# XuanchenLi/Topo4D

Measured on AMD Instinct MI355X. Metric: rasterizer fwd+bwd views/sec, higher is better.
Workload: dtype f32

## Files before the change

topo4d_amd/csrc/t4d_raster.hip:

```cpp
#include <hip/hip_runtime.h>
#include <stdint.h>
#include <stdio.h>
#include <stdlib.h>
#include <string.h>
#include <vector>

#include "../../include/t4d_config.h"
#include "../../include/topo4d_raster.h"
#include "t4d_activations.h"

#define T4D_EXPORT extern "C" __attribute__((visibility("default")))

namespace {

constexpr int kBlock = 256;
#ifndef T4D_FWD_BATCH
#define T4D_FWD_BATCH 192
#endif
constexpr int kFwdBatch = T4D_FWD_BATCH;
#ifndef T4D_BWD_BATCH
#define T4D_BWD_BATCH 128
#endif
constexpr int kBwdBatch = T4D_BWD_BATCH;
constexpr int kSortLdsCap = 2048;
constexpr int kLongBlock = 1024;
constexpr int kScanChunk = 1024;
constexpr int kRankSortMax = 512;
constexpr int kHist = 1024;
constexpr int kBuckets = 24;
constexpr int kGP = T4D_GRAD_PAIR_FLOATS;
constexpr int kCursorSegs = 64;
#ifndef T4D_SEG
// ... 108 lines not shown
    unsigned long long *keys, *sort_tmp;
    float *cut_r2;
    float *final_T;
    uint32_t *n_contrib;
    float *out_color, *out_depth, *out_alpha;
    int32_t *radii;
    const float *dL_dcolor, *dL_ddepth, *dL_dalpha;
    float *grad_pair;
    float *dL_dmeans3D, *dL_dmeans2D, *dL_dcolors, *dL_dshs, *dL_dopacities, *dL_dscales, *dL_drotations, *dL_dcov3D;
    float *tile_dot;
    float *cotangent_dot;
    uint32_t tile_blocks;
    uint32_t fill_blocks;
    uint32_t fill_vec;
    uint4 *slot_tab;
    float *snap;
    uint32_t slots_per_view;
    uint32_t fused_sort;
    unsigned long long *host_status;
    uint32_t seg_min_pairs;
    uint32_t *live;
    uint32_t slots_by_offset;
    uint32_t views_per_set;
};

__device__ __forceinline__ float ndc2pix(float v, int S)
{
#pragma clang fp contract(off)
    return ((v + 1.0f) * S - 1.0f) * 0.5f;
}

__device__ __forceinline__ void tile_rect(float px, float py, int r, int gx, int gy, int &x0, int &y0, int &x1, int &y1)
{
    x0 = min(gx, max(0, (int)((px - r) / T4D_TILE_X)));
    y0 = min(gy, max(0, (int)((py - r) / T4D_TILE_Y)));
    x1 = min(gx, max(0, (int)((px + r + T4D_TILE_X - 1) / T4D_TILE_X)));
    y1 = min(gy, max(0, (int)((py + r + T4D_TILE_Y - 1) / T4D_TILE_Y)));
}

typedef const __attribute__((address_space(4))) float *const_float_p;
struct ViewRecord {
    float view[16], proj[16], campos[3], bg[3], tanx, tany;
};
__device__ __forceinline__ ViewRecord load_view_record(const float *views, const int v)
{
    const_float_p p = (const_float_p)(views + (size_t)v * T4D_VIEW_FLOATS);
    ViewRecord r;
// ... 294 lines not shown
    kp.cut_r2 = reinterpret_cast<float *>(st + L.pair_rank);
    kp.tile_off = reinterpret_cast<uint32_t *>(st + L.tile_off);
    kp.chunk_sum = reinterpret_cast<uint32_t *>(st + L.chunk_sum);
    kp.n_chunks = (kp.T + kScanChunk - 1) / kScanChunk;
    kp.long_bins_elsewhere = (p.flags & T4D_FLAG_NO_LONG_BINS) ? 0 : 1;
    kp.pair_off = reinterpret_cast<uint32_t *>(st + L.pair_off);
    kp.xy = reinterpret_cast<float2 *>(st + L.xy);
    kp.depth = reinterpret_cast<float *>(st + L.depth);
    kp.conic_opacity = reinterpret_cast<float4 *>(st + L.conic_opacity);
    kp.rgb = reinterpret_cast<float *>(st + L.rgb);
    kp.clamped = reinterpret_cast<uint8_t *>(st + L.clamped);
    kp.keys = reinterpret_cast<unsigned long long *>(st + L.keys);
    kp.sort_tmp = reinterpret_cast<unsigned long long *>(st + L.sort_tmp);
    kp.final_T = reinterpret_cast<float *>(st + L.final_T);
    kp.n_contrib = reinterpret_cast<uint32_t *>(st + L.n_contrib);
    kp.slot_tab = reinterpret_cast<uint4 *>(st + L.slot_tab);
    kp.snap = reinterpret_cast<float *>(st + L.snap);
    kp.live = reinterpret_cast<uint32_t *>(st + L.live);
    kp.slots_per_view = seg_capable(p) ? (uint32_t)seg_slots_per_view(p, (size_t)kp.T) : 0u;
    kp.seg_shift = seg_positions(p) == 64 ? 6u : 7u;
    kp.slots_by_offset = seg_mode(p) == 2 ? 1u : 0u;
    kp.seg_min_pairs = seg_mode(p) == 2 ? ((p.flags & T4D_FLAG_NO_LONG_BINS) ? 0xffffffffu : (uint32_t)kSegLongMin) : 0u;
    static_assert(kSegOne == 64 && kSeg == 128, "seg_shift assumes segment lengths of 64 and 128");
}

}

T4D_EXPORT uint32_t t4d_abi_version(void) { return T4D_ABI_VERSION; }
T4D_EXPORT const char *t4d_last_error(void) { return g_err; }

T4D_EXPORT size_t t4d_state_bytes(const T4DProblem *prob)
{
    if (check_problem(prob) != T4D_OK) return 0;
    return make_layout(*prob).total;
}

size_t grad_pair_bytes(const T4DProblem &p) { return align_up((size_t)p.n_views * (size_t)p.pair_capacity * kGP * sizeof(float)); }
size_t tile_dot_bytes(const T4DProblem &p, size_t n_tiles) { return align_up((size_t)p.n_views * n_tiles * 4 * sizeof(float)); }

T4D_EXPORT size_t t4d_backward_scratch_bytes(const T4DProblem *prob)
{
    if (check_problem(prob) != T4D_OK) return 0;
    const size_t n_tiles = (size_t)((prob->W + T4D_TILE_X - 1) / T4D_TILE_X) * ((prob->H + T4D_TILE_Y - 1) / T4D_TILE_Y);
    return grad_pair_bytes(*prob) + tile_dot_bytes(*prob, n_tiles) +
           (prob->sh_coeffs > 0 ? align_up((size_t)prob->n_views * (size_t)prob->P * 3 * sizeof(float)) : 0);
}
// ... 36 lines not shown
{
    int rc = check_problem(prob);
    if (rc != T4D_OK) return rc;
    if (!io || !io->views || !io->means3D || !io->opacities || !io->out_color || !io->out_depth || !io->out_alpha ||
        !io->out_radii || !io->state)
        return fail(T4D_ERR_ARG, "null required pointer in T4DForwardIO");
    if ((io->shs == nullptr) == (io->colors_precomp == nullptr))
        return fail(T4D_ERR_ARG, "provide exactly one of shs / colors_precomp");
    if (io->cov3D_precomp ? (io->scales || io->rotations) : (!io->scales || !io->rotations))
        return fail(T4D_ERR_ARG, "provide exactly one of (scales, rotations) / cov3D_precomp");
    if (io->shs && prob->sh_coeffs < 1) return fail(T4D_ERR_ARG, "shs given but sh_coeffs == 0");
    T4DProblem p = *prob;
    if (!io->shs) p.sh_coeffs = 0;
    const Layout L = make_layout(p);
    if (io->state_bytes < L.total) return fail(T4D_ERR_STATE_SIZE, "state buffer smaller than t4d_state_bytes()");
    hipStream_t stream = (hipStream_t)hip_stream;
    const bool debug = (p.flags & T4D_FLAG_DEBUG_SYNC) != 0;
    const bool checked = debug || (p.flags & T4D_FLAG_CHECKED) != 0;
    char *st = (char *)io->state;

    KP kp;
    memset(&kp, 0, sizeof(kp));
    fill_common(kp, p, L, st);
    kp.views = io->views; kp.means3D = io->means3D; kp.opacities = io->opacities; kp.scales = io->scales;
    kp.rotations = io->rotations; kp.cov3D_precomp = io->cov3D_precomp; kp.colors_precomp = io->colors_precomp;
    kp.shs = io->shs;
    kp.out_color = io->out_color; kp.out_depth = io->out_depth; kp.out_alpha = io->out_alpha; kp.radii = io->out_radii;

    bool status_published = false;
    if (!checked && (p.flags & T4D_FLAG_ASYNC_STATUS) && status && p.n_views == 1 && kp.T <= kSmallTiles &&
        getenv("T4D_NO_SMALL_VIEW") == nullptr && getenv("T4D_STATUS_BY_COPY") == nullptr) {
        void *dptr = nullptr;
        if (hipHostGetDevicePointer(&dptr, (void *)status, 0) == hipSuccess && dptr != nullptr) {
            kp.host_status = (unsigned long long *)dptr;
            status_published = true;
        } else {
            (void)hipGetLastError();
        }
    }
    T4D_HIP(hipMemsetAsync(st, 0, L.zero_end, stream));
    const bool small_view = p.n_views == 1 && kp.T <= kSmallTiles && getenv("T4D_NO_SMALL_VIEW") == nullptr;
    const bool front = small_view && gaussian_grid(p.P, 1) + 1u <= 128u && gaussian_grid(p.P, 1) + 1u <= front_small_resident_blocks() &&
                       getenv("T4D_NO_FRONT_FUSION") == nullptr;
    { ProfScope ps_(stream, K_PREPROCESS);
    if (front) hipLaunchKernelGGL(k_front_small, dim3(gaussian_grid(p.P, 1) + 1), dim3(kBlock), 0, stream, kp);
    else hipLaunchKernelGGL(k_preprocess, dim3(gaussian_grid(p.P, p.n_views)), dim3(kBlock), 0, stream, kp);
// ... 32 lines not shown
    kp.fused_sort = (lat && (p.flags & T4D_FLAG_SHORT_BINS) != 0 && getenv("T4D_NO_FUSED_SORT") == nullptr) ? 1u : 0u;
    const bool long_fwd = kp.slots_per_view != 0u && kp.seg_min_pairs != 0xffffffffu && seg_mode(p) == 2 && !lat && getenv("T4D_NO_LONG_FWD") == nullptr;
    if (long_fwd && getenv("T4D_NO_FUSED_SORT") == nullptr) kp.fused_sort = 1u;
    if (!kp.fused_sort) {
        ProfScope ps_(stream, K_SORT_TILES);
        if (seg_mode(p) == 1 && (p.flags & T4D_FLAG_SHORT_BINS) == 0 && getenv("T4D_SORT_256") == nullptr)
            hipLaunchKernelGGL(k_sort_tiles<kLongBlock>, dim3(min(kp.T * p.n_views, 4 * device_cus())), dim3(kLongBlock), 0, stream, kp);
        else
            hipLaunchKernelGGL(k_sort_tiles<kBlock>, dim3(tile_grid(kp.T * p.n_views, 5, 2)), dim3(kBlock), 0, stream, kp);
    }
    T4D_LAUNCH_CHECK("k_sort_tiles");
    if (kp.long_bins_elsewhere) {
        ProfScope ps_(stream, K_SORT_LONG);
        hipLaunchKernelGGL(k_sort_long_chunks, dim3(min(kp.T * p.n_views, 2 * device_cus())), dim3(kLongBlock), 0, stream, kp);
        hipLaunchKernelGGL(k_merge_long, dim3(min(kp.T * p.n_views, 2 * device_cus())), dim3(kLongBlock), 0, stream, kp);
    }
    T4D_LAUNCH_CHECK("k_sort_long");
    {
    kp.tile_blocks = (uint32_t)(lat ? kp.T * p.n_views : tile_grid(kp.T * p.n_views, 6, 2));
    kp.fill_blocks = (uint32_t)(kp.gy * p.n_views);
    kp.fill_vec = (p.W % 4 == 0 && (((uintptr_t)io->out_color | (uintptr_t)io->out_depth | (uintptr_t)io->out_alpha) & 15u) == 0) ? 1u : 0u;
    if (getenv("T4D_FILL_SCALAR")) kp.fill_vec = 0u;
    const dim3 fgrid(kp.tile_blocks + kp.fill_blocks);
    const bool seg = kp.slots_per_view != 0u && kp.seg_min_pairs != 0xffffffffu;
    const bool seg_one = seg && seg_positions(p) == kSegOne;
    if (long_fwd) {
        { ProfScope ps_(stream, K_RENDER_FWD);
        hipLaunchKernelGGL((k_render_fwd<false, kFwdBatch, 0, true, true>), fgrid, dim3(kBlock), 0, stream, kp);
        }
        T4D_LAUNCH_CHECK("k_render_fwd");
        ProfScope psl_(stream, K_FWD_LONG);
        KP kl = kp;
        kl.tile_blocks = min(kp.slots_per_view, (uint32_t)(8 * device_cus()));
        hipLaunchKernelGGL(k_fwd_long_seg<false>, dim3(kl.tile_blocks), dim3(kBlock), 0, stream, kl);
        T4D_LAUNCH_CHECK("k_fwd_long_seg");
        hipLaunchKernelGGL(k_fwd_long_prefix, dim3(min((uint32_t)kp.T, (uint32_t)(4 * device_cus()))), dim3(kBlock), 0, stream, kl);
        T4D_LAUNCH_CHECK("k_fwd_long_prefix");
        hipLaunchKernelGGL(k_fwd_long_seg<true>, dim3(kl.tile_blocks), dim3(kBlock), 0, stream, kl);
    } else {
    ProfScope ps_(stream, K_RENDER_FWD);
    if (lat) {
        if (seg_one) hipLaunchKernelGGL((k_render_fwd<true, kBlock, kSegOne, true>), fgrid, dim3(kBlock), 0, stream, kp);
        else if (seg) hipLaunchKernelGGL((k_render_fwd<true, kBlock, kSeg, true>), fgrid, dim3(kBlock), 0, stream, kp);
        else hipLaunchKernelGGL((k_render_fwd<true, kBlock, 0, true>), fgrid, dim3(kBlock), 0, stream, kp);
    } else if (seg_one) {
        hipLaunchKernelGGL((k_render_fwd<false, kBlock, kSegOne, true>), fgrid, dim3(kBlock), 0, stream, kp);
// ... 17 lines not shown
    if (!io || !io->views || !io->means3D || !io->opacities || !io->radii || !io->state || !io->dL_dcolor ||
        !io->dL_dmeans3D || !io->dL_dmeans2D || !io->dL_dopacities || !io->scratch)
        return fail(T4D_ERR_ARG, "null required pointer in T4DBackwardIO");
    if ((io->shs == nullptr) == (io->colors_precomp == nullptr))
        return fail(T4D_ERR_ARG, "provide exactly one of shs / colors_precomp");
    if (io->cov3D_precomp ? (io->scales || io->rotations) : (!io->scales || !io->rotations))
        return fail(T4D_ERR_ARG, "provide exactly one of (scales, rotations) / cov3D_precomp");
    if (io->shs ? !io->dL_dshs : !io->dL_dcolors) return fail(T4D_ERR_ARG, "missing colour gradient output");
    if (io->cov3D_precomp ? !io->dL_dcov3D : (!io->dL_dscales || !io->dL_drotations))
        return fail(T4D_ERR_ARG, "missing covariance gradient output");
    T4DProblem p = *prob;
    if (!io->shs) p.sh_coeffs = 0;
    const Layout L = make_layout(p);
    if (io->state_bytes < L.total) return fail(T4D_ERR_STATE_SIZE, "state buffer smaller than t4d_state_bytes()");
    if (io->scratch_bytes < t4d_backward_scratch_bytes(&p))
        return fail(T4D_ERR_STATE_SIZE, "scratch smaller than t4d_backward_scratch_bytes()");
    hipStream_t stream = (hipStream_t)hip_stream;
    const bool debug = (p.flags & T4D_FLAG_DEBUG_SYNC) != 0;
    char *st = (char *)io->state;

    KP kp;
    memset(&kp, 0, sizeof(kp));
    fill_common(kp, p, L, st);
    kp.views = io->views; kp.means3D = io->means3D; kp.opacities = io->opacities; kp.scales = io->scales;
    kp.rotations = io->rotations; kp.cov3D_precomp = io->cov3D_precomp; kp.colors_precomp = io->colors_precomp;
    kp.shs = io->shs;
    kp.radii = const_cast<int32_t *>(io->radii);
    kp.dL_dcolor = io->dL_dcolor; kp.dL_ddepth = io->dL_ddepth; kp.dL_dalpha = io->dL_dalpha;
    kp.grad_pair = (float *)io->scratch;
    if (io->cotangent_dot) {
        kp.tile_dot = (float *)((char *)io->scratch + grad_pair_bytes(p));
        kp.cotangent_dot = io->cotangent_dot;
    }
    kp.dL_dmeans3D = io->dL_dmeans3D; kp.dL_dmeans2D = io->dL_dmeans2D; kp.dL_dcolors = io->dL_dcolors;
    kp.dL_dshs = io->dL_dshs; kp.dL_dopacities = io->dL_dopacities; kp.dL_dscales = io->dL_dscales;
    kp.dL_drotations = io->dL_drotations; kp.dL_dcov3D = io->dL_dcov3D;

    {
    const bool da = kp.dL_ddepth || kp.dL_dalpha;
    const bool lat = latency_launch(kp.T * p.n_views);
    const bool seg_long = seg_mode(p) == 2 && kp.seg_min_pairs != 0xffffffffu && getenv("T4D_NO_SEGMENTS") == nullptr;
    const bool seg = seg_mode(p) == 1 && getenv("T4D_NO_SEGMENTS") == nullptr;
    kp.tile_blocks = seg ? (uint32_t)p.n_views * kp.slots_per_view
                         : (uint32_t)(lat ? kp.T * p.n_views : tile_grid(kp.T * p.n_views, 4, 2));
    uint32_t grid = kp.tile_blocks + (kp.tile_dot ? (uint32_t)p.n_views * ((kp.T + kEmptySpan - 1) / kEmptySpan) : 0u);
#define T4D_BWD_LAUNCH(DA_, LAT_, SEG_) hipLaunchKernelGGL((k_render_bwd<DA_, LAT_, SEG_>), dim3(grid), dim3(kBlock), 0, stream, kp)
// ... 119 lines not shown
```

topo4d_amd/csrc/t4d_raster_render_bwd.h:

```cpp
__device__ __forceinline__ void tile_pixel_bwd(int tid, int tx, int ty, int &px, int &py)
{
    const int w = tid >> 6, r = (tid >> 4) & 3, i = tid & 15;
    px = tx * T4D_TILE_X + ((w & 1) << 3) + ((r & 1) << 2) + (i >> 2);
    py = ty * T4D_TILE_Y + ((w >> 1) << 3) + ((r >> 1) << 2) + (i & 3);
}

__device__ __forceinline__ int fwd_thread_of(int tid) { return (tid & ~15) | ((tid & 3) << 2) | ((tid >> 2) & 3); }

struct RowWeights { float X, ks, kg; };

__device__ __forceinline__ RowWeights row_weights(const int lane)
{
    const int r = lane >> 4, i = lane & 15, bank = i >> 2, b1 = (i >> 1) & 1;
    RowWeights k;
    k.X = (float)(((r & 1) << 2) + (i >> 2)) - 3.5f;
    const float y0 = (float)((r >> 1) << 2) - 3.5f;
    const float Y = y0 + (float)(i & 3), Yp = y0 + (float)((i & 3) ^ 2);
    auto Ka = [&](float y) { return bank == 1 ? y * y : (bank == 3 ? 0.f : 1.f); };
    auto Kb = [&](float y) { return (bank & 1) ? 0.f : y; };
    k.ks = b1 ? Kb(Y) : Ka(Y);
    k.kg = b1 ? Kb(Yp) : Ka(Yp);
    return k;
}

// ... 33 lines not shown
        float d;
        asm(T4D_RED_X
            "v_add_f32_dpp %[d], %[v6], %[v6] row_ror:8 row_mask:0xf bank_mask:0xf\n\t"
            T4D_RED_X4
            "v_add_f32_dpp %[d], %[d], %[d] row_ror:4 row_mask:0xf bank_mask:0xf\n\t"
            "v_cndmask_b32_e64 %[c], %[d], %[a], %[m1]\n\t"
            "v_cndmask_b32_e64 %[d], %[a], %[d], %[m1]\n\t"
            "v_mul_f32_e32 %[a], %[b], %[ks]\n\t"
            "v_fmac_f32_dpp %[a], %[b], %[kg] quad_perm:[2,3,0,1] row_mask:0xf bank_mask:0xf\n\t"
            "v_add_f32_dpp %[d], %[c], %[d] quad_perm:[2,3,0,1] row_mask:0xf bank_mask:0xf\n\t"
            "v_cndmask_b32_e64 %[b], %[d], %[a], %[m0]\n\t"
            "v_cndmask_b32_e64 %[a], %[a], %[d], %[m0]\n\t"
            "s_nop 0\n\t"
            "v_add_f32_dpp %[a], %[b], %[a] quad_perm:[1,0,3,2] row_mask:0xf bank_mask:0xf"
            : T4D_RED_OUT, [d] "=&v"(d) : T4D_RED_IN, [v6] "v"(cd), [m1] "s"(0xccccccccccccccccull));
        return a;
    }
#undef T4D_RED_X
#undef T4D_RED_X4
#undef T4D_RED_OUT
#undef T4D_RED_IN
}

__device__ __forceinline__ int row10_index(const int lane)
{
    const int b0 = lane & 1, b1 = (lane >> 1) & 1, bank = (lane >> 2) & 3;
    if (!b0) {
        if (bank == 0) return b1 ? 2 : 0;
        if (bank == 1) return b1 ? -1 : 5;
        if (bank == 2) return b1 ? 4 : 1;
        return -1;
    }
    if (!b1) return bank == 0 ? 3 : (bank == 1 ? 7 : (bank == 2 ? 6 : 8));
    return bank == 0 ? 9 : -1;
}

__device__ __forceinline__ void moments_about_centre(float (&m)[10], const float pxf, const float pyf)
{
    const double px = pxf, py = pyf, M00 = m[0], M10 = m[1], M01 = m[2], M20 = m[3], M11 = m[4], M02 = m[5];
    const double sx = fma(px, M00, -M10), sy = fma(py, M00, -M01);
    m[1] = (float)sx; m[2] = (float)sy;
    m[3] = (float)fma(px, sx, -fma(px, M10, -M20));
    m[4] = (float)fma(px, sy, -fma(py, M10, -M11));
    m[5] = (float)fma(py, sy, -fma(py, M01, -M02));
}

__device__ __forceinline__ float moment_e(const float e) { return __uint_as_float(__float_as_uint(e) & 0xffffffc0u); }

__device__ __forceinline__ uint32_t row_max_u32(uint32_t v)
{
    v = max(v, (uint32_t)__builtin_amdgcn_update_dpp(0, (int)v, 0xB1, 0xf, 0xf, true));
    v = max(v, (uint32_t)__builtin_amdgcn_update_dpp(0, (int)v, 0x4E, 0xf, 0xf, true));
    v = max(v, (uint32_t)__builtin_amdgcn_update_dpp(0, (int)v, 0x141, 0xf, 0xf, true));
    v = max(v, (uint32_t)__builtin_amdgcn_update_dpp(0, (int)v, 0x140, 0xf, 0xf, true));
    return v;
}

#ifndef T4D_BWD_WAVES
#define T4D_BWD_WAVES 5
#endif
#ifndef T4D_SEG_WAVES
#define T4D_SEG_WAVES 5
#endif
#ifndef T4D_BWD_DA_WAVES
#define T4D_BWD_DA_WAVES T4D_BWD_WAVES
#endif
#define T4D_BWD_NW (LAT ? 2 : (SEGN != 0 ? T4D_SEG_WAVES : (DA ? T4D_BWD_DA_WAVES : T4D_BWD_WAVES)))
#define T4D_BWD_ATTR __attribute__((amdgpu_waves_per_eu(LAT ? 1 : T4D_BWD_NW, T4D_BWD_NW)))
constexpr int kAcc = 10;
constexpr int kEmptySpan = 64;
template <bool DA, bool LAT, int SEGN, bool LONG = false>
__global__ __launch_bounds__(kBlock) T4D_BWD_ATTR void k_render_bwd(const KP kp)
{
    constexpr bool SEG = SEGN != 0;
    constexpr int kSeg = SEG ? SEGN : ::kSeg;
    constexpr int kBwdBatch = SEG ? SEGN : ::kBwdBatch;
    constexpr int kSlabs = LAT ? 16 : 4;
    constexpr int kChunks = (kBwdBatch + 63) / 64;
    constexpr int kListStride = kBwdBatch + 4;
    constexpr int kEnt = 40;
    static_assert(kBwdBatch % 64 == 0, "staged slots come in chunks of one per lane");
    static_assert(kGP == kAcc, "the slab entry and the scratch record hold the same ten sums");
    static_assert(kAcc * 4 == kEnt, "a slab entry and a staged record must have the same stride");
    struct __attribute__((aligned(16))) Shared {
        unsigned char rec[(kBwdBatch + 1) * kEnt];
        float acc[kSlabs][kBwdBatch + 1][kAcc];
        unsigned short list[4][4][kListStride];
        float cut_r2[kChunks * 64];
        uint32_t pair[kBwdBatch];
        uint32_t wmax[4];
    };
    static_assert(((kBwdBatch + 1) * kEnt) % 8 == 0 && (sizeof(float) * kSlabs * (kBwdBatch + 1) * kAcc) % 8 == 0 &&
                  (sizeof(unsigned short) * 16 * kListStride) % 8 == 0, "8-byte members must stay 8-byte aligned");
    __shared__ Shared sh;
    auto &s_rec = sh.rec;
    auto &s_pair = sh.pair;
    auto &s_acc = sh.acc;
    auto &s_r2 = sh.cut_r2;
    auto &s_wmax = sh.wmax;
    auto &s_list = sh.list;
    constexpr int kNull = kBwdBatch;

    const int tid = threadIdx.x;
    const int wave = __builtin_amdgcn_readfirstlane(tid >> 6), lane = tid & 63, row = lane >> 4;
    const int my_slot = (!DA && row10_index(lane & 15) == 9) ? -1 : row10_index(lane & 15);
    const RowWeights rw = row_weights(lane);
    if (tid == 0) {
#pragma unroll
        for (int k = 0; k < kEnt / 8; k++) reinterpret_cast<float2 *>(s_rec + kNull * kEnt)[k] = make_float2(0.f, 0.f);
    }
    if (blockIdx.x >= kp.tile_blocks) {
        const uint32_t spans = (uint32_t)(kp.T + kEmptySpan - 1) / kEmptySpan;
        const uint32_t j = blockIdx.x - kp.tile_blocks;
        const int v = (int)(j / spans), t0 = (int)(j % spans) * kEmptySpan;
        const float *vb = kp.views + (size_t)v * T4D_VIEW_FLOATS + 35;
        const float b0 = vb[0], b1 = vb[1], b2 = vb[2];
        if (b0 == 0.f && b1 == 0.f && b2 == 0.f) return;
        const size_t HWe = (size_t)kp.H * kp.W;
        const float *dc = kp.dL_dcolor + (size_t)v * 3 * HWe;
        for (int t = t0; t < min(t0 + kEmptySpan, kp.T); t++) {
            if (kp.tile_count[(size_t)v * kp.T + t] != 0u) continue;
            const int ty = t / kp.gx, tx = t - ty * kp.gx;
            int ex, ey;
            tile_pixel(tid, tx, ty, ex, ey);
            float d = 0.f;
            if (ex < kp.W && ey < kp.H) {
                const size_t pe = (size_t)ey * kp.W + ex;
                d = fmaf(b0, dc[pe], fmaf(b1, dc[HWe + pe], b2 * dc[2 * HWe + pe]));
            }
            d = wave_sum_to_lane63(d);
            if (lane == 63) kp.tile_dot[((size_t)v * kp.T + t) * 4 + wave] = d;
        }
        return;
    }
    uint4 it;
    if (SEG && !LONG) {
        it = kp.slot_tab[blockIdx.x];
        if (it.w == 0u) return;
    }
    for (int i = tid; i < kSlabs * (kBwdBatch + 1) * kAcc; i += kBlock) (&s_acc[0][0][0])[i] = 0.f;
    for (uint32_t item = blockIdx.x; item < (SEG ? (LONG ? kp.status->live_segments : blockIdx.x + 1u) : (uint32_t)(kp.V * kp.T)); item += kp.tile_blocks) {
    if (SEG && LONG) it = kp.slot_tab[kp.live[item]];
    if (!SEG) it = kp.items[item];
    const int seg_j = SEG ? (int)(it.w & 0x7fffffffu) : 0;
    const int v = (int)(it.x >> 20), t_ = (int)(it.x & 0xfffffu);
    const int ty = t_ / kp.gx, tx = t_ - ty * kp.gx;
    const uint32_t off = it.y, n = it.z;
    if (n == 0) break;
    if (!SEG && LONG && n >= kp.seg_min_pairs &&
        kp.slot_tab[(size_t)v * kp.slots_per_view + seg_slot0(kp, off, (uint32_t)t_)].w != 0u) continue;
    const unsigned long long *keys = kp.keys + (size_t)v * kp.cap + off;
    const float *r2_in = kp.cut_r2 + (size_t)v * kp.cap + off;
    const float2 *xy = kp.xy + (size_t)v * kp.P;
    const float4 *co = kp.conic_opacity + (size_t)v * kp.P;
    const float *rgb = kp.shs ? kp.rgb + (size_t)v * kp.P * 3 : kp.colors_precomp + 3 * param_row0(kp, v);
    const int32_t *radii = kp.radii + (size_t)v * kp.P;
    const uint32_t *pair_off = kp.pair_off + (size_t)v * kp.P;
    float2 *grad_pair = reinterpret_cast<float2 *>(kp.grad_pair) + (size_t)v * kp.cap * (kGP / 2);
    const float *vr = kp.views + (size_t)v * T4D_VIEW_FLOATS;

    int px, py;
    tile_pixel_bwd(tid, tx, ty, px, py);
    const bool inside = px < kp.W && py < kp.H;
    const v2f pix_f = { (float)px, (float)py };
    const size_t HW = (size_t)kp.H * kp.W, pix = (size_t)py * kp.W + px;

    float T_final = 0.f, dp0 = 0.f, dp1 = 0.f, dp2 = 0.f, ddep = 0.f, dalp = 0.f;
    uint32_t last_contributor = 0;
    if (inside) {
        T_final = kp.final_T[(size_t)v * HW + pix];
        last_contributor = kp.n_contrib[(size_t)v * HW + pix];
        const float *dc = kp.dL_dcolor + (size_t)v * 3 * HW;
        dp0 = dc[pix]; dp1 = dc[HW + pix]; dp2 = dc[2 * HW + pix];
        if (DA && kp.dL_ddepth) ddep = kp.dL_ddepth[(size_t)v * HW + pix];
        if (DA && kp.dL_dalpha) dalp = kp.dL_dalpha[(size_t)v * HW + pix];
    }
    const v2f dp01 = { dp0, dp1 };
    float T = T_final;
    float acc = vr[35] * dp0 + vr[36] * dp1 + vr[37] * dp2;
    const int nb = (int)((n + kBwdBatch - 1) / kBwdBatch);
    if (SEG && seg_j + 1 < nb) {
        const uint32_t p = (uint32_t)(seg_j + 1) * kSeg;
        if (last_contributor > p) {
            const float *sb = kp.snap + ((size_t)v * kp.slots_per_view + seg_slot0(kp, off, (uint32_t)t_)) * (kSnapFloats * kBlock) + fwd_thread_of(tid);
            const float *sp = sb + (size_t)seg_j * (kSnapFloats * kBlock), *sf = sb + (size_t)(nb - 1) * (kSnapFloats * kBlock);
            const float Tp = sp[0];
            float suf = fmaf(sf[kBlock] - sp[kBlock], dp0, fmaf(sf[2 * kBlock] - sp[2 * kBlock], dp1, (sf[3 * kBlock] - sp[3 * kBlock]) * dp2));
            if (DA) suf = fmaf(sf[4 * kBlock] - sp[4 * kBlock], ddep, suf) + (Tp - T_final) * dalp;
            acc = fmaf(T_final, acc, suf) / Tp;
            T = Tp;
        }
    }

    const uint32_t rmax_v = row_max_u32(last_contributor);
    uint32_t row_max[4];
#pragma unroll
    for (int r = 0; r < 4; r++) row_max[r] = lane_value(rmax_v, 16 * r);
    const uint32_t wave_max = max(max(row_max[0], row_max[1]), max(row_max[2], row_max[3]));
// ... 178 lines not shown
#pragma unroll
                for (int s = 0; s < kSlabs / 4; s++) {
                    float2 *src = reinterpret_cast<float2 *>(&s_acc[w * (kSlabs / 4) + s][tid][0]);
#pragma unroll
                    for (int k = 0; k < 5; k++) {
                        const float2 b2 = src[k];
                        m[2 * k] += b2.x; m[2 * k + 1] += b2.y;
                        src[k] = make_float2(0.f, 0.f);
                    }
                }
                moments_about_centre(m, pc.x - ((float)(tx * T4D_TILE_X + ((w & 1) << 3)) + 3.5f),
                                        pc.y - ((float)(ty * T4D_TILE_Y + ((w >> 1) << 3)) + 3.5f));
#pragma unroll
                for (int k = 0; k < 10; k++) a[k] += m[k];
            }
            const uint32_t pr = s_pair[tid];
            if (pr < kp.cap) {
#pragma unroll
                for (int k = 0; k < kGP / 2; k++) grad_pair[(size_t)pr * (kGP / 2) + k] = make_float2(a[2 * k], a[2 * k + 1]);
            }
        }
        __syncthreads();
    }
    if (kp.tile_dot && seg_j == 0) {
        const float d = wave_sum_to_lane63(acc);
        if (lane == 63) kp.tile_dot[((size_t)v * kp.T + t_) * 4 + wave] = d;
    }
    }
}
```

topo4d_amd/csrc/t4d_raster_render_fwd.h:

```cpp
constexpr float kLog2e = 1.4426950408889634f;


__device__ __forceinline__ void tile_pixel(int tid, int tx, int ty, int &px, int &py)
{
    const int w = tid >> 6, r = (tid >> 4) & 3, i = tid & 15;
    px = tx * T4D_TILE_X + ((w & 1) << 3) + ((r & 1) << 2) + (i & 3);
    py = ty * T4D_TILE_Y + ((w >> 1) << 3) + ((r >> 1) << 2) + (i >> 2);
}

__device__ __forceinline__ float cutoff_radius2(const float4 co)
{
    const float lnarg = __logf(255.0f * co.w);
    if (!(lnarg > -1e-3f)) return -1.0f;
    const float mid = 0.5f * (co.x + co.z);
    const float det = co.x * co.z - co.y * co.y;
    const float disc = mid * mid - det;
    const float lmin = det * __builtin_amdgcn_rcpf(mid + __builtin_amdgcn_sqrtf(fmaxf(disc, 0.f)));
    if (!(lmin > 0.f) || !(mid > 0.f)) return __builtin_huge_valf();
    return 2.0f * (lnarg + 2e-3f) * __builtin_amdgcn_rcpf(lmin) * 1.001f;
}

__device__ __forceinline__ void wave_touch_masks(const float2 p, const float r2, const int tx, const int ty, const int w,
                                                 unsigned long long (&out)[4])
{
// ... 46 lines not shown
    for (int cc = 0; cc < NCHUNK; cc++) {
        const int c = REVERSE ? NCHUNK - 1 - cc : cc;
        const unsigned long long mw = m[c];
        if (mw == 0ull) continue;
        const int below = (int)__builtin_amdgcn_mbcnt_hi((uint32_t)(mw >> 32), __builtin_amdgcn_mbcnt_lo((uint32_t)mw, 0u));
        const int tot = __builtin_popcountll(mw);
        if (__builtin_amdgcn_inverse_ballot_w64(mw)) list[cnt + (REVERSE ? tot - 1 - below : below)] = (unsigned short)((((c + chunk0) << 6) + lane) * SCALE);
        cnt += tot;
    }
    return cnt;
}

template <int GROUP = 4>
__device__ __forceinline__ void pad_visit_list(unsigned short *list, const int cnt, const int nsteps, const int lane,
                                               const unsigned short null_entry)
{
#pragma clang loop vectorize(disable) unroll(disable)
    for (int p2 = cnt + lane; p2 < nsteps + GROUP - 1; p2 += 64) list[p2] = null_entry;
}

__device__ __forceinline__ void fill_empty_tile_row(const KP &kp, const uint32_t j)
{
    const int tid = threadIdx.x;
    const int v = (int)(j / (uint32_t)kp.gy), ty = (int)(j - (uint32_t)v * (uint32_t)kp.gy);
    const uint32_t *tc = kp.tile_count + (size_t)v * kp.T + (size_t)ty * kp.gx;
    const float *vr = kp.views + (size_t)v * T4D_VIEW_FLOATS;
    const float b0 = vr[35], b1 = vr[36], b2 = vr[37];
    const int y0 = ty * T4D_TILE_Y, rows = min(T4D_TILE_Y, kp.H - y0);
    const size_t HW = (size_t)kp.H * kp.W;
    float *oc = kp.out_color + (size_t)v * 3 * HW + (size_t)y0 * kp.W;
    float *od = kp.out_depth + (size_t)v * HW + (size_t)y0 * kp.W;
    float *oa = kp.out_alpha + (size_t)v * HW + (size_t)y0 * kp.W;
    if (kp.fill_vec) {
        const int qw = kp.W >> 2;
        int r = tid / qw, q = tid - r * qw;
        const int dr = kBlock / qw, dq = kBlock - dr * qw;
        while (r < rows) {
            if (tc[q >> 2] == 0u) {
                const size_t o = (size_t)r * kp.W + 4 * q;
                *reinterpret_cast<float4 *>(oc + o) = make_float4(b0, b0, b0, b0);
                *reinterpret_cast<float4 *>(oc + HW + o) = make_float4(b1, b1, b1, b1);
                *reinterpret_cast<float4 *>(oc + 2 * HW + o) = make_float4(b2, b2, b2, b2);
                *reinterpret_cast<float4 *>(od + o) = make_float4(0.f, 0.f, 0.f, 0.f);
                *reinterpret_cast<float4 *>(oa + o) = make_float4(0.f, 0.f, 0.f, 0.f);
            }
            r += dr; q += dq;
            if (q >= qw) { q -= qw; r++; }
// ... 34 lines not shown
    static_assert(kFB <= kBlock && kFB % 64 == 0 && kFB % kSub == 0, "one staging thread per slot (it clears the slot when the list is shorter)");
    constexpr bool FUSE = LONG;
    constexpr int kRecBytes = ((kFB + 1) * kRec + 15) / 16 * 16;
    unsigned char *s_rec;
    unsigned short (*s_list)[4][kListStride];
    unsigned long long *s_sort;
    if constexpr (FUSE) {
        constexpr int kStage = kRecBytes + 4 * 4 * kListStride * 2;
        constexpr int kRaw = kStage < kSortLdsCap * 8 ? kSortLdsCap * 8 : kStage;
        __shared__ __attribute__((aligned(16))) unsigned char s_raw[kRaw];
        s_rec = s_raw;
        s_list = reinterpret_cast<unsigned short (*)[4][kListStride]>(s_raw + kRecBytes);
        s_sort = reinterpret_cast<unsigned long long *>(s_raw);
    } else {
        __shared__ __attribute__((aligned(16))) unsigned char s_rec_[(kFB + 1) * kRec];
        __shared__ __attribute__((aligned(8))) unsigned short s_list_[4][4][kListStride];
        __shared__ unsigned long long s_sort_[LAT ? kSortLdsCap : 1];
        s_rec = s_rec_; s_list = s_list_; s_sort = s_sort_;
    }
    __shared__ uint32_t s_wave_done[4];
    const int tid = threadIdx.x;
    const int wave = tid >> 6, lane = tid & 63, row = lane >> 4;
    const uint32_t total_blocks = kp.tile_blocks + kp.fill_blocks;
    const uint32_t fills_before = (uint32_t)(((unsigned long long)blockIdx.x * kp.fill_blocks) / total_blocks);
    if ((uint32_t)(((unsigned long long)(blockIdx.x + 1u) * kp.fill_blocks) / total_blocks) != fills_before) {
        fill_empty_tile_row(kp, fills_before);
        return;
    }
    if constexpr (FUSE) {
        if (kp.fused_sort) {
            for (uint32_t item = blockIdx.x - fills_before; item < (uint32_t)(kp.V * kp.T); item += kp.tile_blocks) {
                const uint4 it = kp.items[item];
                if (it.w == 0u) break;
                if (it.z > 1u) {
                    sort_one_bin<false, kBlock>(kp, (int)(it.x >> 20), it.y, it.z, s_sort, tid, wave, lane);
                    __syncthreads();
                }
            }
            __threadfence_block();
            __syncthreads();
        }
    }
    if (tid < kRec / 4) reinterpret_cast<float *>(s_rec + kNull * kRec)[tid] = 0.f;
    for (uint32_t item = blockIdx.x - fills_before; item < (uint32_t)(kp.V * kp.T); item += kp.tile_blocks) {
    const uint4 it = kp.items[item];
    if (it.w == 0u) break;
    const int v = (int)(it.x >> 20), t_ = (int)(it.x & 0xfffffu);
    const int ty = t_ / kp.gx, tx = t_ - ty * kp.gx;
    const uint32_t off = it.y, n = it.z;
    if (LONG && n >= kp.seg_min_pairs) continue;
    const unsigned long long *keys = kp.keys + (size_t)v * kp.cap + off;
    float *r2_out = kp.cut_r2 + (size_t)v * kp.cap + off;
    const float2 *xy = kp.xy + (size_t)v * kp.P;
    const float4 *co = kp.conic_opacity + (size_t)v * kp.P;
    const float *rgb = kp.shs ? kp.rgb + (size_t)v * kp.P * 3 : kp.colors_precomp + 3 * param_row0(kp, v);
    float *snap = nullptr;
    if (SEG && n > (uint32_t)kSeg && n >= kp.seg_min_pairs)
        snap = kp.snap + ((size_t)v * kp.slots_per_view + seg_slot0(kp, off, (uint32_t)t_)) * (kSnapFloats * kBlock) + tid;

    int px, py;
    tile_pixel(tid, tx, ty, px, py);
    const bool inside = px < kp.W && py < kp.H;
    const v2f pix_f = { (float)px, (float)py };
    const float *vr = kp.views + (size_t)v * T4D_VIEW_FLOATS;
    const float bg0 = __uint_as_float(__builtin_amdgcn_readfirstlane(__float_as_uint(vr[35])));
    const float bg1 = __uint_as_float(__builtin_amdgcn_readfirstlane(__float_as_uint(vr[36])));
    const float bg2 = __uint_as_float(__builtin_amdgcn_readfirstlane(__float_as_uint(vr[37])));
    unsigned long long done_m = __ballot(!inside);
    uint32_t gate = inside ? 0xffffffffu : 0u;
    float T = 1.0f, C0 = 0.f, C1 = 0.f, C2 = 0.f, D = 0.f;
    uint32_t last_contributor = 0;

    bool keys_lds = false;
    unsigned long long k_cur = ~0ull, k_nxt = ~0ull;
    float2 pre_p = make_float2(0.f, 0.f);
    float4 pre_c = make_float4(0.f, 0.f, 0.f, 0.f);
    float pre_r0 = 0.f, pre_r1 = 0.f, pre_r2 = 0.f;
    if (LAT) {
        static_assert(!LAT || kFB == kBlock, "the latency build stages one splat per thread");
        if (kp.fused_sort) {
            sort_one_bin<true, kBlock>(kp, v, off, n, s_sort, tid, wave, lane);
            __threadfence_block();
            __syncthreads();
            keys_lds = n <= (uint32_t)kSortLdsCap;
        }
        if ((uint32_t)tid < n) k_cur = keys_lds ? s_sort[tid] : keys[tid];
        if ((uint32_t)(kFB + tid) < n) k_nxt = keys_lds ? s_sort[kFB + tid] : keys[kFB + tid];
// ... 139 lines not shown
                const float4 cd = LAT ? cds[u] : *reinterpret_cast<const float4 *>(s_rec + e[u] + 32);
                const float w = ok ? alpha[u] * T : 0.f;
                C0 = fmaf(cd.x, w, C0); C1 = fmaf(cd.y, w, C1); C2 = fmaf(cd.z, w, C2);
                D = fmaf(cd.w, w, D);
                T = ok ? test_T : T;
                last_e = ok ? e[u] : last_e;
            }
            if (done_m == ~0ull) break;
        }
        if (SEG) {
            if (done_m == ~0ull) break;
            if (snap != nullptr && sub_lo + (uint32_t)kSeg < n) {
                float *sp = snap + (size_t)(sub_lo / kSeg) * (kSnapFloats * kBlock);
                sp[0] = T; sp[kBlock] = C0; sp[2 * kBlock] = C1; sp[3 * kBlock] = C2; sp[4 * kBlock] = D;
            }
        }
        }
        if (last_e != 0xffffffffu) last_contributor = b + ((last_e * 43691u) >> 21) + 1u;
    }
    if (SEG && snap != nullptr) {
        float *sp = snap + (size_t)((n - 1u) / kSeg) * (kSnapFloats * kBlock);
        sp[0] = T; sp[kBlock] = C0; sp[2 * kBlock] = C1; sp[3 * kBlock] = C2; sp[4 * kBlock] = D;
    }
    if (inside) {
        const size_t HW = (size_t)kp.H * kp.W, pix = (size_t)py * kp.W + px;
        if (n != 0) {
            kp.final_T[(size_t)v * HW + pix] = T;
            kp.n_contrib[(size_t)v * HW + pix] = last_contributor;
        }
        float *oc = kp.out_color + (size_t)v * 3 * HW;
        oc[pix] = C0 + T * bg0;
        oc[HW + pix] = C1 + T * bg1;
        oc[2 * HW + pix] = C2 + T * bg2;
        kp.out_depth[(size_t)v * HW + pix] = D;
        kp.out_alpha[(size_t)v * HW + pix] = 1.f - T;
    }
    __syncthreads();
    }
}
```

Baseline: 56900.

## Replace integer divisions with precomputed multipliers and read kernel args directly

```diff
diff --git a/topo4d_amd/csrc/t4d_raster.hip b/topo4d_amd/csrc/t4d_raster.hip
--- a/topo4d_amd/csrc/t4d_raster.hip
+++ b/topo4d_amd/csrc/t4d_raster.hip
@@ -8,6 +8,7 @@
 #include "../../include/t4d_config.h"
 #include "../../include/topo4d_raster.h"
 #include "t4d_activations.h"
+#include "t4d_tile_div.h"
 
 #define T4D_EXPORT extern "C" __attribute__((visibility("default")))
 
@@ -162,7 +163,21 @@
     uint32_t *live;
     uint32_t slots_by_offset;
     uint32_t views_per_set;
+    T4DDiv div_gx;
+    T4DDiv div_gy;
+    T4DDiv div_spans;
+    T4DDiv div_blocks;
+    uint32_t div_blocks_ok;
+    uint32_t div_ok;
 };
+
+typedef const __attribute__((address_space(4))) KP *kp_kernarg_p;
+__device__ __forceinline__ kp_kernarg_p kernarg_kp()
+{
+    kp_kernarg_p p = (kp_kernarg_p)__builtin_amdgcn_kernarg_segment_ptr();
+    asm volatile("" : "+s"(p));
+    return p;
+}
 
 __device__ __forceinline__ float ndc2pix(float v, int S)
 {
@@ -503,6 +518,9 @@
     kp.slots_by_offset = seg_mode(p) == 2 ? 1u : 0u;
     kp.seg_min_pairs = seg_mode(p) == 2 ? ((p.flags & T4D_FLAG_NO_LONG_BINS) ? 0xffffffffu : (uint32_t)kSegLongMin) : 0u;
     static_assert(kSegOne == 64 && kSeg == 128, "seg_shift assumes segment lengths of 64 and 128");
+    kp.div_ok = (t4d_div_make((uint32_t)kp.gx, (uint64_t)kp.T, kp.div_gx) &&
+                 t4d_div_make((uint32_t)kp.gy, (uint64_t)kp.V * (uint64_t)kp.gy, kp.div_gy) &&
+                 t4d_div_make(empty_spans(kp.T), (uint64_t)kp.V * empty_spans(kp.T), kp.div_spans)) ? 1u : 0u;
 }
 
 }
@@ -585,6 +603,7 @@
     KP kp;
     memset(&kp, 0, sizeof(kp));
     fill_common(kp, p, L, st);
+    if (!kp.div_ok) return fail(T4D_ERR_ARG, "no exact multiplier for this tile grid");
     kp.views = io->views; kp.means3D = io->means3D; kp.opacities = io->opacities; kp.scales = io->scales;
     kp.rotations = io->rotations; kp.cov3D_precomp = io->cov3D_precomp; kp.colors_precomp = io->colors_precomp;
     kp.shs = io->shs;
@@ -663,6 +682,10 @@
     kp.fill_vec = (p.W % 4 == 0 && (((uintptr_t)io->out_color | (uintptr_t)io->out_depth | (uintptr_t)io->out_alpha) & 15u) == 0) ? 1u : 0u;
     if (getenv("T4D_FILL_SCALAR")) kp.fill_vec = 0u;
     const dim3 fgrid(kp.tile_blocks + kp.fill_blocks);
+    {
+        const uint64_t top = (uint64_t)fgrid.x * kp.fill_blocks;
+        kp.div_blocks_ok = (top < (1ull << 32) && t4d_div_make(fgrid.x, top + 1u, kp.div_blocks)) ? 1u : 0u;
+    }
     const bool seg = kp.slots_per_view != 0u && kp.seg_min_pairs != 0xffffffffu;
     const bool seg_one = seg && seg_positions(p) == kSegOne;
     if (long_fwd) {
@@ -726,6 +749,7 @@
     KP kp;
     memset(&kp, 0, sizeof(kp));
     fill_common(kp, p, L, st);
+    if (!kp.div_ok) return fail(T4D_ERR_ARG, "no exact multiplier for this tile grid");
     kp.views = io->views; kp.means3D = io->means3D; kp.opacities = io->opacities; kp.scales = io->scales;
     kp.rotations = io->rotations; kp.cov3D_precomp = io->cov3D_precomp; kp.colors_precomp = io->colors_precomp;
     kp.shs = io->shs;
diff --git a/topo4d_amd/csrc/t4d_raster_render_bwd.h b/topo4d_amd/csrc/t4d_raster_render_bwd.h
--- a/topo4d_amd/csrc/t4d_raster_render_bwd.h
+++ b/topo4d_amd/csrc/t4d_raster_render_bwd.h
@@ -79,7 +79,7 @@
 #undef T4D_RED_IN
 }
 
-__device__ __forceinline__ int row10_index(const int lane)
+constexpr int row10_index(const int lane)
 {
     const int b0 = lane & 1, b1 = (lane >> 1) & 1, bank = (lane >> 2) & 3;
     if (!b0) {
@@ -90,6 +90,17 @@
     }
     if (!b1) return bank == 0 ? 3 : (bank == 1 ? 7 : (bank == 2 ? 6 : 8));
     return bank == 0 ? 9 : -1;
+}
+
+template <bool NINE>
+constexpr unsigned long long row10_table()
+{
+    unsigned long long t = 0ull;
+    for (int i = 0; i < 16; i++) {
+        const int s = row10_index(i);
+        t |= (unsigned long long)((NINE && s == 9) ? 0 : s + 1) << (4 * i);
+    }
+    return t;
 }
 
 __device__ __forceinline__ void moments_about_centre(float (&m)[10], const float pxf, const float pyf)
@@ -126,6 +137,7 @@
 #define T4D_BWD_ATTR __attribute__((amdgpu_waves_per_eu(LAT ? 1 : T4D_BWD_NW, T4D_BWD_NW)))
 constexpr int kAcc = 10;
 constexpr int kEmptySpan = 64;
+__host__ __device__ inline uint32_t empty_spans(const int T) { return (uint32_t)(T + kEmptySpan - 1) / kEmptySpan; }
 template <bool DA, bool LAT, int SEGN, bool LONG = false>
 __global__ __launch_bounds__(kBlock) T4D_BWD_ATTR void k_render_bwd(const KP kp)
 {
@@ -158,18 +170,24 @@
     auto &s_list = sh.list;
     constexpr int kNull = kBwdBatch;
 
+    uint4 it = make_uint4(0u, 0u, 0u, 0u);
+    if (!SEG && blockIdx.x < kp.tile_blocks) {
+        it = kp.items[blockIdx.x];
+        if (it.z == 0u) return;
+    }
     const int tid = threadIdx.x;
     const int wave = __builtin_amdgcn_readfirstlane(tid >> 6), lane = tid & 63, row = lane >> 4;
-    const int my_slot = (!DA && row10_index(lane & 15) == 9) ? -1 : row10_index(lane & 15);
+    constexpr unsigned long long kSlotTable = row10_table<!DA>();
+    const int my_slot = (int)((uint32_t)(kSlotTable >> (4 * (lane & 15))) & 15u) - 1;
     const RowWeights rw = row_weights(lane);
     if (tid == 0) {
 #pragma unroll
         for (int k = 0; k < kEnt / 8; k++) reinterpret_cast<float2 *>(s_rec + kNull * kEnt)[k] = make_float2(0.f, 0.f);
     }
     if (blockIdx.x >= kp.tile_blocks) {
-        const uint32_t spans = (uint32_t)(kp.T + kEmptySpan - 1) / kEmptySpan;
+        const uint32_t spans = empty_spans(kp.T);
         const uint32_t j = blockIdx.x - kp.tile_blocks;
-        const int v = (int)(j / spans), t0 = (int)(j % spans) * kEmptySpan;
+        const int v = (int)t4d_div(j, kp.div_spans), t0 = (int)(j - (uint32_t)v * spans) * kEmptySpan;
         const float *vb = kp.views + (size_t)v * T4D_VIEW_FLOATS + 35;
         const float b0 = vb[0], b1 = vb[1], b2 = vb[2];
         if (b0 == 0.f && b1 == 0.f && b2 == 0.f) return;
@@ -177,7 +195,7 @@
         const float *dc = kp.dL_dcolor + (size_t)v * 3 * HWe;
         for (int t = t0; t < min(t0 + kEmptySpan, kp.T); t++) {
             if (kp.tile_count[(size_t)v * kp.T + t] != 0u) continue;
-            const int ty = t / kp.gx, tx = t - ty * kp.gx;
+            const int ty = (int)t4d_div((uint32_t)t, kp.div_gx), tx = t - ty * kp.gx;
             int ex, ey;
             tile_pixel(tid, tx, ty, ex, ey);
             float d = 0.f;
@@ -190,47 +208,54 @@
         }
         return;
     }
-    uint4 it;
     if (SEG && !LONG) {
         it = kp.slot_tab[blockIdx.x];
         if (it.w == 0u) return;
     }
-    for (int i = tid; i < kSlabs * (kBwdBatch + 1) * kAcc; i += kBlock) (&s_acc[0][0][0])[i] = 0.f;
+    {
+        constexpr int kPairs = kSlabs * (kBwdBatch + 1) * kAcc / 2;
+        static_assert(kAcc % 2 == 0, "slab entries are cleared as float2");
+        float2 *a2 = reinterpret_cast<float2 *>(&s_acc[0][0][0]);
+#pragma unroll
+        for (int i = 0; i < kPairs / kBlock; i++) a2[i * kBlock + tid] = make_float2(0.f, 0.f);
+        if (tid < kPairs % kBlock) a2[(kPairs / kBlock) * kBlock + tid] = make_float2(0.f, 0.f);
+    }
     for (uint32_t item = blockIdx.x; item < (SEG ? (LONG ? kp.status->live_segments : blockIdx.x + 1u) : (uint32_t)(kp.V * kp.T)); item += kp.tile_blocks) {
     if (SEG && LONG) it = kp.slot_tab[kp.live[item]];
-    if (!SEG) it = kp.items[item];
+    if (!SEG && item != blockIdx.x) it = kp.items[item];
     const int seg_j = SEG ? (int)(it.w & 0x7fffffffu) : 0;
     const int v = (int)(it.x >> 20), t_ = (int)(it.x & 0xfffffu);
-    const int ty = t_ / kp.gx, tx = t_ - ty * kp.gx;
+    const int ty = (int)t4d_div((uint32_t)t_, kp.div_gx), tx = t_ - ty * kp.gx;
     const uint32_t off = it.y, n = it.z;
     if (n == 0) break;
     if (!SEG && LONG && n >= kp.seg_min_pairs &&
         kp.slot_tab[(size_t)v * kp.slots_per_view + seg_slot0(kp, off, (uint32_t)t_)].w != 0u) continue;
-    const unsigned long long *keys = kp.keys + (size_t)v * kp.cap + off;
-    const float *r2_in = kp.cut_r2 + (size_t)v * kp.cap + off;
-    const float2 *xy = kp.xy + (size_t)v * kp.P;
-    const float4 *co = kp.conic_opacity + (size_t)v * kp.P;
-    const float *rgb = kp.shs ? kp.rgb + (size_t)v * kp.P * 3 : kp.colors_precomp + 3 * param_row0(kp, v);
-    const int32_t *radii = kp.radii + (size_t)v * kp.P;
-    const uint32_t *pair_off = kp.pair_off + (size_t)v * kp.P;
-    float2 *grad_pair = reinterpret_cast<float2 *>(kp.grad_pair) + (size_t)v * kp.cap * (kGP / 2);
-    const float *vr = kp.views + (size_t)v * T4D_VIEW_FLOATS;
+    const kp_kernarg_p kt = kernarg_kp();
+    const unsigned long long *keys = kt->keys + (size_t)v * kt->cap + off;
+    const float *r2_in = kt->cut_r2 + (size_t)v * kt->cap + off;
+    const float2 *xy = kt->xy + (size_t)v * kt->P;
+    const float4 *co = kt->conic_opacity + (size_t)v * kt->P;
+    const float *rgb = kt->shs ? kt->rgb + (size_t)v * kt->P * 3 : kt->colors_precomp + 3 * param_row0(kp, v);
+    const int32_t *radii = kt->radii + (size_t)v * kt->P;
+    const uint32_t *pair_off = kt->pair_off + (size_t)v * kt->P;
+    float2 *grad_pair = reinterpret_cast<float2 *>(kt->grad_pair) + (size_t)v * kt->cap * (kGP / 2);
+    const float *vr = kt->views + (size_t)v * T4D_VIEW_FLOATS;
 
     int px, py;
     tile_pixel_bwd(tid, tx, ty, px, py);
-    const bool inside = px < kp.W && py < kp.H;
+    const bool inside = px < kt->W && py < kt->H;
     const v2f pix_f = { (float)px, (float)py };
-    const size_t HW = (size_t)kp.H * kp.W, pix = (size_t)py * kp.W + px;
+    const size_t HW = (size_t)kt->H * kt->W, pix = (size_t)py * kt->W + px;
 
     float T_final = 0.f, dp0 = 0.f, dp1 = 0.f, dp2 = 0.f, ddep = 0.f, dalp = 0.f;
     uint32_t last_contributor = 0;
     if (inside) {
-        T_final = kp.final_T[(size_t)v * HW + pix];
-        last_contributor = kp.n_contrib[(size_t)v * HW + pix];
-        const float *dc = kp.dL_dcolor + (size_t)v * 3 * HW;
+        T_final = kt->final_T[(size_t)v * HW + pix];
+        last_contributor = kt->n_contrib[(size_t)v * HW + pix];
+        const float *dc = kt->dL_dcolor + (size_t)v * 3 * HW;
         dp0 = dc[pix]; dp1 = dc[HW + pix]; dp2 = dc[2 * HW + pix];
-        if (DA && kp.dL_ddepth) ddep = kp.dL_ddepth[(size_t)v * HW + pix];
-        if (DA && kp.dL_dalpha) dalp = kp.dL_dalpha[(size_t)v * HW + pix];
+        if (DA && kt->dL_ddepth) ddep = kt->dL_ddepth[(size_t)v * HW + pix];
+        if (DA && kt->dL_dalpha) dalp = kt->dL_dalpha[(size_t)v * HW + pix];
     }
     const v2f dp01 = { dp0, dp1 };
     float T = T_final;
@@ -455,9 +480,10 @@
         }
         __syncthreads();
     }
-    if (kp.tile_dot && seg_j == 0) {
+    const kp_kernarg_p ke = kernarg_kp();
+    if (ke->tile_dot && seg_j == 0) {
         const float d = wave_sum_to_lane63(acc);
-        if (lane == 63) kp.tile_dot[((size_t)v * kp.T + t_) * 4 + wave] = d;
-    }
-    }
-}
+        if (lane == 63) ke->tile_dot[((size_t)v * ke->T + t_) * 4 + wave] = d;
+    }
+    }
+}
diff --git a/topo4d_amd/csrc/t4d_raster_render_fwd.h b/topo4d_amd/csrc/t4d_raster_render_fwd.h
--- a/topo4d_amd/csrc/t4d_raster_render_fwd.h
+++ b/topo4d_amd/csrc/t4d_raster_render_fwd.h
@@ -92,7 +92,7 @@
 __device__ __forceinline__ void fill_empty_tile_row(const KP &kp, const uint32_t j)
 {
     const int tid = threadIdx.x;
-    const int v = (int)(j / (uint32_t)kp.gy), ty = (int)(j - (uint32_t)v * (uint32_t)kp.gy);
+    const int v = (int)t4d_div(j, kp.div_gy), ty = (int)(j - (uint32_t)v * (uint32_t)kp.gy);
     const uint32_t *tc = kp.tile_count + (size_t)v * kp.T + (size_t)ty * kp.gx;
     const float *vr = kp.views + (size_t)v * T4D_VIEW_FLOATS;
     const float b0 = vr[35], b1 = vr[36], b2 = vr[37];
@@ -173,8 +173,15 @@
     const int tid = threadIdx.x;
     const int wave = tid >> 6, lane = tid & 63, row = lane >> 4;
     const uint32_t total_blocks = kp.tile_blocks + kp.fill_blocks;
-    const uint32_t fills_before = (uint32_t)(((unsigned long long)blockIdx.x * kp.fill_blocks) / total_blocks);
-    if ((uint32_t)(((unsigned long long)(blockIdx.x + 1u) * kp.fill_blocks) / total_blocks) != fills_before) {
+    uint32_t fills_before, fills_through;
+    if (kp.div_blocks_ok) {
+        fills_before = t4d_div(blockIdx.x * kp.fill_blocks, kp.div_blocks);
+        fills_through = t4d_div((blockIdx.x + 1u) * kp.fill_blocks, kp.div_blocks);
+    } else {
+        fills_before = (uint32_t)(((unsigned long long)blockIdx.x * kp.fill_blocks) / total_blocks);
+        fills_through = (uint32_t)(((unsigned long long)(blockIdx.x + 1u) * kp.fill_blocks) / total_blocks);
+    }
+    if (fills_through != fills_before) {
         fill_empty_tile_row(kp, fills_before);
         return;
     }
@@ -197,23 +204,24 @@
     const uint4 it = kp.items[item];
     if (it.w == 0u) break;
     const int v = (int)(it.x >> 20), t_ = (int)(it.x & 0xfffffu);
-    const int ty = t_ / kp.gx, tx = t_ - ty * kp.gx;
+    const int ty = (int)t4d_div((uint32_t)t_, kp.div_gx), tx = t_ - ty * kp.gx;
     const uint32_t off = it.y, n = it.z;
     if (LONG && n >= kp.seg_min_pairs) continue;
-    const unsigned long long *keys = kp.keys + (size_t)v * kp.cap + off;
-    float *r2_out = kp.cut_r2 + (size_t)v * kp.cap + off;
-    const float2 *xy = kp.xy + (size_t)v * kp.P;
-    const float4 *co = kp.conic_opacity + (size_t)v * kp.P;
-    const float *rgb = kp.shs ? kp.rgb + (size_t)v * kp.P * 3 : kp.colors_precomp + 3 * param_row0(kp, v);
+    const kp_kernarg_p kt = kernarg_kp();
+    const unsigned long long *keys = kt->keys + (size_t)v * kt->cap + off;
+    float *r2_out = kt->cut_r2 + (size_t)v * kt->cap + off;
+    const float2 *xy = kt->xy + (size_t)v * kt->P;
+    const float4 *co = kt->conic_opacity + (size_t)v * kt->P;
+    const float *rgb = kt->shs ? kt->rgb + (size_t)v * kt->P * 3 : kt->colors_precomp + 3 * param_row0(kp, v);
     float *snap = nullptr;
-    if (SEG && n > (uint32_t)kSeg && n >= kp.seg_min_pairs)
-        snap = kp.snap + ((size_t)v * kp.slots_per_view + seg_slot0(kp, off, (uint32_t)t_)) * (kSnapFloats * kBlock) + tid;
+    if (SEG && n > (uint32_t)kSeg && n >= kt->seg_min_pairs)
+        snap = kt->snap + ((size_t)v * kt->slots_per_view + seg_slot0(kp, off, (uint32_t)t_)) * (kSnapFloats * kBlock) + tid;
 
     int px, py;
     tile_pixel(tid, tx, ty, px, py);
-    const bool inside = px < kp.W && py < kp.H;
+    const bool inside = px < kt->W && py < kt->H;
     const v2f pix_f = { (float)px, (float)py };
-    const float *vr = kp.views + (size_t)v * T4D_VIEW_FLOATS;
+    const float *vr = kt->views + (size_t)v * T4D_VIEW_FLOATS;
     const float bg0 = __uint_as_float(__builtin_amdgcn_readfirstlane(__float_as_uint(vr[35])));
     const float bg1 = __uint_as_float(__builtin_amdgcn_readfirstlane(__float_as_uint(vr[36])));
     const float bg2 = __uint_as_float(__builtin_amdgcn_readfirstlane(__float_as_uint(vr[37])));
@@ -399,18 +407,19 @@
         float *sp = snap + (size_t)((n - 1u) / kSeg) * (kSnapFloats * kBlock);
         sp[0] = T; sp[kBlock] = C0; sp[2 * kBlock] = C1; sp[3 * kBlock] = C2; sp[4 * kBlock] = D;
     }
+    const kp_kernarg_p ke = kernarg_kp();
     if (inside) {
-        const size_t HW = (size_t)kp.H * kp.W, pix = (size_t)py * kp.W + px;
+        const size_t HW = (size_t)ke->H * ke->W, pix = (size_t)py * ke->W + px;
         if (n != 0) {
-            kp.final_T[(size_t)v * HW + pix] = T;
-            kp.n_contrib[(size_t)v * HW + pix] = last_contributor;
-        }
-        float *oc = kp.out_color + (size_t)v * 3 * HW;
+            ke->final_T[(size_t)v * HW + pix] = T;
+            ke->n_contrib[(size_t)v * HW + pix] = last_contributor;
+        }
+        float *oc = ke->out_color + (size_t)v * 3 * HW;
         oc[pix] = C0 + T * bg0;
         oc[HW + pix] = C1 + T * bg1;
         oc[2 * HW + pix] = C2 + T * bg2;
-        kp.out_depth[(size_t)v * HW + pix] = D;
-        kp.out_alpha[(size_t)v * HW + pix] = 1.f - T;
+        ke->out_depth[(size_t)v * HW + pix] = D;
+        ke->out_alpha[(size_t)v * HW + pix] = 1.f - T;
     }
     __syncthreads();
     }
diff --git a/topo4d_amd/csrc/t4d_tile_div.h b/topo4d_amd/csrc/t4d_tile_div.h
--- /dev/null
+++ b/topo4d_amd/csrc/t4d_tile_div.h
@@ -0,0 +1,34 @@
+#pragma once
+#include <stdint.h>
+
+#if defined(__HIPCC__) || defined(__CUDACC__)
+#define T4D_HD __host__ __device__
+#else
+#define T4D_HD
+#endif
+
+struct T4DDiv {
+    uint32_t mul;
+    uint32_t shift;
+};
+
+inline bool t4d_div_make(const uint32_t d, const uint64_t limit, T4DDiv &r)
+{
+    r.mul = 0u; r.shift = 0u;
+    if (d == 1u) return true;
+    if (d == 0u || limit > (1ull << 32)) return false;
+    bool found = false;
+    const uint64_t tmax = limit ? limit - 1u : 0u;
+    for (uint32_t s = 0; s < 32u; s++) {
+        const uint64_t pow = 1ull << (32u + s);
+        const uint64_t m = (pow + d - 1u) / d;
+        if (m >> 32) break;
+        const uint64_t e = m * d - pow;
+        if (tmax * e < pow) { r.mul = (uint32_t)m; r.shift = s; found = true; }
+    }
+    return found;
+}
+
+T4D_HD inline uint32_t t4d_div_mulhi(const uint32_t a, const uint32_t b) { return (uint32_t)(((uint64_t)a * b) >> 32); }
+
+T4D_HD inline uint32_t t4d_div(const uint32_t t, const T4DDiv dv) { return dv.mul ? (t4d_div_mulhi(t, dv.mul) >> dv.shift) : t; }
```

After: 59240 (median of 6 runs). +4.1%, better.
